# andrewendlinger/xmris

Hardware: AMD Instinct MI355X
Metric: spectra/sec (zero_fill->apodize->FFT->autophase), n_time=4096; HBM-roofline % (higher is better)
Workload: dtype f32

## Files before the change

xmris_amd/csrc/xm_coarse.h:

```cpp
#pragma once
#include "xm_kernels.h"

typedef _Float16 xm_h8 __attribute__((ext_vector_type(8)));
typedef _Float16 xm_h2 __attribute__((ext_vector_type(2)));
typedef float xm_f16v __attribute__((ext_vector_type(16)));

struct CoarseArgs {
  const void* in;
  const float* window;
  const Cx<float>* w1024;
  float* est;
  unsigned long long* gkey;
  long long in_stride;
  long long n_batch;
  float scale2;
};

constexpr int kCoarseWaves = 4;

XM_DEV Cx<float> coarse_w1024(const Cx<float>* __restrict__ t, unsigned k) {
  k &= 1023u;
  const Cx<float> w = t[k & 511u];
  return (k & 512u) ? mk<float>(-w.re, -w.im) : w;
}

XM_DEV xm_h8 coarse_pack(const float* v) {
  union {
    xm_h8 v8;
    xm_h2 v2[4];
  } u;
#pragma unroll
  for (int j = 0; j < 4; ++j) {
    const xm_f2 p = {v[2 * j], v[2 * j + 1]};
    u.v2[j] = __builtin_convertvector(p, xm_h2);
  }
  return u.v8;
}

template <bool IN64>
__global__ __launch_bounds__(64 * kCoarseWaves, 2) void k_coarse_mfma(CoarseArgs A) {
  const unsigned lane = threadIdx.x & 63u, r = lane & 31u, h = lane >> 5;
  const long long wave = (long long)blockIdx.x * kCoarseWaves + (threadIdx.x >> 6);
  const long long n_waves = (long long)gridDim.x * kCoarseWaves;

  xm_h8 b1r, b1i, b1n, a2r[2], a2i[2], a2n[2];
  {
    float cr[8], ci[8], cn[8];
#pragma unroll
    for (int j = 0; j < 8; ++j) {
      const Cx<float> w = coarse_w1024(A.w1024, 32u * ((8u * h + (unsigned)j) * r));
      cr[j] = w.re;
      ci[j] = w.im;
      cn[j] = -w.im;
    }
    b1r = coarse_pack(cr);
    b1i = coarse_pack(ci);
    b1n = coarse_pack(cn);
#pragma unroll
    for (int s = 0; s < 2; ++s) {
#pragma unroll
      for (int j = 0; j < 8; ++j) {
        const unsigned n2 = 16u * s + 8u * ((unsigned)j >> 2) + 4u * h + ((unsigned)j & 3u);
        const Cx<float> w = coarse_w1024(A.w1024, 32u * (n2 * r));
        cr[j] = w.re;
        ci[j] = w.im;
        cn[j] = -w.im;
      }
      a2r[s] = coarse_pack(cr);
      a2i[s] = coarse_pack(ci);
      a2n[s] = coarse_pack(cn);
    }
  }
  float twr[16], twi[16];
#pragma unroll
  for (int q = 0; q < 16; ++q) {
    const unsigned n2 = ((unsigned)q & 3u) + 8u * ((unsigned)q >> 2) + 4u * h;
    const Cx<float> w = coarse_w1024(A.w1024, n2 * r);
    twr[q] = w.re;
    twi[q] = w.im;
  }
  float wnd[8];
#pragma unroll
  for (int j = 0; j < 8; ++j) wnd[j] = A.window[32u * (8u * h + (unsigned)j) + r];

  auto fetch = [&](long long s, Cx<float>* x) {
    if constexpr (IN64) {
      const xm_d2* __restrict__ row = reinterpret_cast<const xm_d2*>(A.in) + s * A.in_stride;
#pragma unroll
      for (int j = 0; j < 8; ++j) {
        const xm_d2 v = __builtin_nontemporal_load(row + 32u * (8u * h + (unsigned)j) + r);
        x[j] = mk<float>((float)v.x, (float)v.y);
      }
      return;
    }
    const xm_f2* __restrict__ row = reinterpret_cast<const xm_f2*>(A.in) + s * A.in_stride;
#pragma unroll
    for (int j = 0; j < 8; ++j) {
      const xm_f2 v = __builtin_nontemporal_load(row + 32u * (8u * h + (unsigned)j) + r);
      x[j] = mk<float>(v.x, v.y);
    }
  };

  unsigned best_key = 0u, best_row = 0u;
  bool have = false;
  constexpr int DEPTH = 1;
  Cx<float> nx[DEPTH][8];
  long long s = wave;
#pragma unroll
  for (int d = 0; d < DEPTH; ++d)
    if (s + d * n_waves < A.n_batch) fetch(s + d * n_waves, nx[d]);
  auto one_row = [&](Cx<float>* cur, long long s) {
    float re[8], im[8];
    float m = 0.f;
#pragma unroll
    for (int j = 0; j < 8; ++j) {
      re[j] = cur[j].re * wnd[j];
      im[j] = cur[j].im * wnd[j];
      m = fmaxf(m, fmaxf(fabsf(re[j]), fabsf(im[j])));
    }
    if (s + DEPTH * n_waves < A.n_batch) fetch(s + DEPTH * n_waves, cur);
    unsigned e = (wave_reduce_u32<true>(__float_as_uint(m)) >> 23) & 0xffu;
    e = e > 253u ? 253u : (e < 1u ? 1u : e);
    const float up = __uint_as_float((254u - e) << 23);
    const float down = __uint_as_float(e << 23);
#pragma unroll
    for (int j = 0; j < 8; ++j) {
      re[j] *= up;
      im[j] *= up;
    }
    const xm_h8 ar = coarse_pack(re), ai = coarse_pack(im);
    xm_f16v d1r = {0.f}, d1i = {0.f};
    d1r = __builtin_amdgcn_mfma_f32_32x32x16_f16(ar, b1r, d1r, 0, 0, 0);
    d1r = __builtin_amdgcn_mfma_f32_32x32x16_f16(ai, b1n, d1r, 0, 0, 0);
    d1i = __builtin_amdgcn_mfma_f32_32x32x16_f16(ar, b1i, d1i, 0, 0, 0);
    d1i = __builtin_amdgcn_mfma_f32_32x32x16_f16(ai, b1r, d1i, 0, 0, 0);
    float zr[16], zi[16];
#pragma unroll
    for (int q = 0; q < 16; ++q) {
      zr[q] = d1r[q] * twr[q] - d1i[q] * twi[q];
      zi[q] = d1r[q] * twi[q] + d1i[q] * twr[q];
    }
    xm_f16v d2r = {0.f}, d2i = {0.f};
#pragma unroll
    for (int k = 0; k < 2; ++k) {
      const xm_h8 br = coarse_pack(zr + 8 * k), bi = coarse_pack(zi + 8 * k);
      d2r = __builtin_amdgcn_mfma_f32_32x32x16_f16(a2r[k], br, d2r, 0, 0, 0);
      d2r = __builtin_amdgcn_mfma_f32_32x32x16_f16(a2n[k], bi, d2r, 0, 0, 0);
      d2i = __builtin_amdgcn_mfma_f32_32x32x16_f16(a2r[k], bi, d2i, 0, 0, 0);
      d2i = __builtin_amdgcn_mfma_f32_32x32x16_f16(a2i[k], br, d2i, 0, 0, 0);
    }
    float bv = -1.f;
#pragma unroll
    for (int q = 0; q < 16; ++q) bv = fmaxf(bv, d2r[q] * d2r[q] + d2i[q] * d2i[q]);
    bv = amax_nan_if_unset(bv);
    bv = bv * (down * down) * A.scale2;
    const unsigned key = wave_reduce_u32<true>(bv != bv ? 0x7fc00000u : __float_as_uint(bv));
    const unsigned row = (unsigned)s;
    const bool take = !have || key > best_key;
    best_key = take ? key : best_key;
    best_row = take ? row : best_row;
    have = true;
    if (lane == 0u) A.est[s] = __uint_as_float(key);
  };
  for (; s < A.n_batch; s += DEPTH * n_waves) {
#pragma unroll
    for (int d = 0; d < DEPTH; ++d)
      if (s + d * n_waves < A.n_batch) one_row(nx[d], s + d * n_waves);
  }
  if (A.gkey && have && lane == 0u)
    atomicMax(A.gkey + (blockIdx.x % XM_KEY_SLOTS) * XM_KEY_STRIDE,
              ((unsigned long long)best_key << 32) | (unsigned long long)(0xffffffffu - best_row));
}
```

xmris_amd/csrc/xm_zf2p.h:

```cpp
#pragma once
#include "xm_kernels.h"

enum { ZF2P_LOAD16 = 1, ZF2P_NT = 2, ZF2P_QUEUE = 8, ZF2P_EST = 16, ZF2P_CAND = 32, ZF2P_IN64 = 64 };
constexpr int ZF2P_CAND_CAP = 16;
constexpr int ZF2P_CAND_KMAX = 16384;
constexpr int ZF2P_CAND_ROWS = 1, ZF2P_CAND_EST = 1 + ZF2P_CAND_CAP, ZF2P_CAND_COUNT = 1 + 2 * ZF2P_CAND_CAP,
              ZF2P_CAND_TOP = ZF2P_CAND_COUNT + 1, ZF2P_CAND_BITMAP = ZF2P_CAND_TOP + 1;
constexpr size_t zf2p_cand_lds_bytes() { return (ZF2P_CAND_BITMAP + ZF2P_CAND_KMAX / 32) * sizeof(unsigned); }

constexpr int xm_ilog2(int v) {
  int s = 0;
  while ((1 << s) < v) ++s;
  return s;
}

template <class PL, bool L16>
constexpr int zf2p_pad_shift() {
  if (!L16) return -1;
  return PL::radix(0) == 8 ? 4 : xm_ilog2(2 * PL::radix(0));
}

template <class PL, int MODE, int OPT>
__global__ __launch_bounds__(PL::NT, (zf2_waves<float, PL>())) void k_zf2p(PipeArgs<float> A) {
  using T = float;
  using V = xm_f2;
  constexpr unsigned N = 2 * PL::N, NT = PL::NT;
  constexpr int P = PL::P;
  constexpr bool WRITE = (MODE & ZF2_WRITE) != 0, PHASE = (MODE & ZF2_PHASE) != 0, AMAX = (MODE & ZF2_AMAX) != 0;
  constexpr bool RAMP = (MODE & ZF2_RAMP) != 0;
  constexpr bool L16 = (OPT & ZF2P_LOAD16) != 0;
  constexpr int AUX = (OPT & ZF2P_NT) ? 2 : 0;
  constexpr bool EST = (OPT & ZF2P_EST) != 0, CAND = (OPT & ZF2P_CAND) != 0, IN64 = (OPT & ZF2P_IN64) != 0;
  static_assert(!EST || (NT == XM_WAVE && AMAX && !WRITE), "the per-row estimate is stored by the row's one wave");
  static_assert(!CAND || (AMAX && !WRITE && (OPT & ZF2P_QUEUE) == 0), "candidates: maxima only, static order");
  static_assert(!(IN64 && L16), "pair loads are complex64 loads");
  static_assert(!(PHASE && RAMP), "phase table and ramp are exclusive");
  static_assert(!RAMP || WRITE, "a ramp needs an output");
  static_assert(P % 2 == 0 && NT >= XM_WAVE, "pair loads need an even number of points per thread, whole waves");
  using FFT = BlockFFT<V, PL, zf2p_pad_shift<PL, L16>()>;
  using HT = HotTw<T, PL, RAMP>;
  extern __shared__ __attribute__((aligned(16))) char xm_smem[];
  Cx<V>* lds = reinterpret_cast<Cx<V>*>(xm_smem);
  Cx<T>* mid = reinterpret_cast<Cx<T>*>(lds + FFT::lds_elems());
  T* red_v = reinterpret_cast<T*>(mid + HT::mid_lds_size());
  int* red_i = reinterpret_cast<int*>(red_v + NT / XM_WAVE + 1);
  unsigned* lds_next = reinterpret_cast<unsigned*>(red_i + NT / XM_WAVE + 1);
  constexpr bool QUEUE = (OPT & ZF2P_QUEUE) != 0;
  const unsigned t = threadIdx.x;
  const unsigned lane = t & (XM_WAVE - 1), half = lane >> 5;
  const unsigned col = L16 ? (t & ~(XM_WAVE - 1u)) + 2u * (lane & 31u) + half : t;

  long long n_rows = A.n_batch;
  unsigned* cand = lds_next + ZF2P_CAND_ROWS;
  const unsigned n_in = (unsigned)A.n_in;
  if constexpr (CAND) {
    float* cand_e = reinterpret_cast<float*>(lds_next + ZF2P_CAND_EST);
    unsigned* cand_n = lds_next + ZF2P_CAND_COUNT;
    unsigned* top_bits = lds_next + ZF2P_CAND_TOP;
    unsigned* bitmap = lds_next + ZF2P_CAND_BITMAP;
    const unsigned G = gridDim.x, b = blockIdx.x;
    const unsigned kmax = (unsigned)((A.n_batch + G - 1) / G);
    for (unsigned i = t; i < (kmax + 31u) / 32u; i += NT) bitmap[i] = 0u;
    if (t < XM_WAVE) {
      const unsigned long long k = __hip_atomic_load(A.gkey_in + t * XM_KEY_STRIDE, __ATOMIC_RELAXED, __HIP_MEMORY_SCOPE_AGENT);
      const unsigned hi = wave_reduce_u32<true>((unsigned)(k >> 32));
      if (t == 0) *top_bits = hi;
    }
    __syncthreads();
    const float thr = A.band2 * __uint_as_float(*top_bits);
    for (unsigned k = t; k < kmax; k += NT) {
      const long long r = (long long)k * G + (b + 37u * k) % G;
      if (r < A.n_batch) {
        const float e = A.est[r];
        if (e >= thr || e != e) atomicOr(&bitmap[k >> 5], 1u << (k & 31u));
      }
    }
    __syncthreads();
    if (t == 0) {
      unsigned n = 0;
      for (unsigned w = 0; w < (kmax + 31u) / 32u; ++w) {
        unsigned bits = bitmap[w];
        while (bits) {
          const unsigned k = w * 32u + (unsigned)__builtin_ctz(bits);
          bits &= bits - 1u;
          const unsigned r = (unsigned)((long long)k * G + (b + 37u * k) % G);
          float e = A.est[r];
          e = e != e ? __builtin_inff() : e;
// ... 8 lines not shown
          cand[pos] = r;
          cand_e[pos] = e;
          n = n < (unsigned)ZF2P_CAND_CAP ? n + 1u : n;
        }
      }
      *cand_n = n;
    }
    __syncthreads();
    n_rows = (long long)(unsigned)__builtin_amdgcn_readfirstlane((int)*cand_n);
  }
  const bool live = !CAND || n_rows > 0;

  HT tw;
  tw.mid = HT::mid_in_lds() ? mid : A.tw;
  if (live) {
    tw.load(A.tw, (int)t);
    for (unsigned i = t; i < (unsigned)HT::mid_lds_size(); i += NT) mid[i] = A.tw[i];
  }
  if constexpr (RAMP) {
    double sn, cs;
    sincos(A.ramp_db * (double)(2u * t), &sn, &cs);
    tw.fold(mk<T>((T)cs, (T)sn));
  }
  Cx<T> rot = live ? A.aux[col] : mk<T>(T(0), T(0));
  if constexpr (RAMP) rot = rot * mk<T>(A.ramp_e[0], A.ramp_e[1]);
  const unsigned coff = col - (unsigned)A.pad_left;
  T w[P];
#pragma unroll
  for (int q = 0; q < P; ++q) {
    const bool ok = live && (coff + NT * q) < n_in;
    w[q] = ok ? (A.window ? A.window[col + NT * q] * A.scale : A.scale) : T(0);
  }
  __syncthreads();

  constexpr int NRAW = L16 ? P / 2 : P;
  typedef unsigned raw_t __attribute__((ext_vector_type((L16 || IN64) ? 4 : 2)));
  raw_t raw[NRAW];
  const unsigned e0 = (t & ~(XM_WAVE - 1u)) + 2u * (lane & 31u) + NT * half - (unsigned)A.pad_left;
  auto fetch = [&](long long s2, unsigned ee0, unsigned cc, unsigned nin) {
    constexpr size_t EB = IN64 ? 16u : 8u;
    const char* __restrict__ row = reinterpret_cast<const char*>(A.in) + (size_t)(s2 * A.in_stride) * EB;
    if constexpr (L16) {
#pragma unroll
      for (int j = 0; j < P / 2; ++j) {
        const unsigned e = min(ee0 + 2u * NT * j, nin - 2u);
        raw[j] = __builtin_nontemporal_load(reinterpret_cast<const raw_t*>(row + (size_t)e * 8u));
      }
    } else {
#pragma unroll
      for (int q = 0; q < P; ++q) {
        const unsigned e = min(cc + NT * q, nin - 1u);
        raw[q] = *reinterpret_cast<const raw_t*>(row + (size_t)e * EB);
      }
    }
  };
  unsigned best_key = 0, best_row = 0;
  bool have = false;
  auto rowid = [&](long long v) -> long long {
    if constexpr (CAND) return (long long)(unsigned)__builtin_amdgcn_readfirstlane((int)cand[v]);
    else return v;
  };
  unsigned gb_seen = 0;
  auto next_live = [&](long long v) -> long long {
    if constexpr (CAND) {
      const float* cand_e = reinterpret_cast<const float*>(lds_next + ZF2P_CAND_EST);
      const unsigned gb = wave_reduce_u32<true>(__hip_atomic_load(A.gbest + lane * (2u * XM_KEY_STRIDE), __ATOMIC_RELAXED,
                                                                  __HIP_MEMORY_SCOPE_AGENT));
      gb_seen = gb;
      const float lim = A.band2 * __uint_as_float(gb);
      while (v < n_rows && __uint_as_float((unsigned)__builtin_amdgcn_readfirstlane((int)__float_as_uint(cand_e[v]))) < lim) ++v;
    }
    return v;
  };
  const long long ch = (!CAND && A.queue_chunk > 0) ? A.queue_chunk : 1;
  const long long c_first = CAND ? 0 : blockIdx.x, c_step = CAND ? 1 : gridDim.x;
  long long c_cur = c_first, c_nxt = c_cur + c_step, c_nn = c_nxt + c_step;
  long long s = c_cur * ch;
  unsigned off = 0;
  if constexpr (CAND) {
    if (n_rows > 0) {
      const float* cand_e = reinterpret_cast<const float*>(lds_next + ZF2P_CAND_EST);
      const float top = __uint_as_float((unsigned)__builtin_amdgcn_readfirstlane((int)__float_as_uint(cand_e[0])));
      const float emax2 = __uint_as_float((unsigned)__builtin_amdgcn_readfirstlane((int)lds_next[ZF2P_CAND_TOP]));
      if (top < 0.81f * emax2) {
#pragma unroll 1
        for (int i = 0; i < 3; ++i) __builtin_amdgcn_s_sleep(127);
        if (t < XM_WAVE) {
          const long long nx = next_live(0);
          if (t == 0u) *lds_next = (unsigned)nx;
        }
        __syncthreads();
        s = (long long)(unsigned)__builtin_amdgcn_readfirstlane((int)*lds_next);
        __syncthreads();
      }
    }
  }
  if (s < n_rows) fetch(rowid(s), e0, coff, n_in);
  if constexpr (QUEUE) {
    if (t == 0) *lds_next = atomicAdd(A.queue, 1u) + gridDim.x;
    __syncthreads();
    c_nxt = (long long)(unsigned)__builtin_amdgcn_readfirstlane((int)*lds_next);
    __syncthreads();
  }

  while (s < n_rows) {
    const bool chunk_end = (off + 1 == (unsigned)ch) || (s + 1 >= n_rows);
    long long s_nxt = chunk_end ? c_nxt * ch : s + 1;
    unsigned tt = t, cc = col, sh = (unsigned)A.out_shift, nin = n_in, pl = (unsigned)A.pad_left, ee0 = e0;
    asm volatile("" : "+v"(tt));
    asm volatile("" : "+v"(cc));
    asm volatile("" : "+v"(ee0));
    asm volatile("" : "+s"(sh));
    asm volatile("" : "+s"(nin));
    asm volatile("" : "+s"(pl));

    Cx<T> xr[P];
    if constexpr (L16) {
#pragma unroll
      for (int j = 0; j < P / 2; ++j) {
        const auto re = __builtin_amdgcn_permlane32_swap(raw[j].x, raw[j].z, false, false);
        const auto im = __builtin_amdgcn_permlane32_swap(raw[j].y, raw[j].w, false, false);
        xr[2 * j] = mk<T>(__uint_as_float(re[0]), __uint_as_float(im[0]));
        xr[2 * j + 1] = mk<T>(__uint_as_float(re[1]), __uint_as_float(im[1]));
      }
    } else if constexpr (IN64) {
#pragma unroll
      for (int q = 0; q < P; ++q) {
        Cx<double> d;
        __builtin_memcpy(&d, &raw[q], 16);
        xr[q] = mk<T>((T)d.re, (T)d.im);
      }
    } else {
#pragma unroll
      for (int q = 0; q < P; ++q) xr[q] = mk<T>(__uint_as_float(raw[q].x), __uint_as_float(raw[q].y));
    }
    Cx<V> v[P];
    static_for<0, P>([&](auto qc) {
      constexpr int q = decltype(qc)::value;
      const Cx<T> e = xr[q] * w[q];
      const Cx<T> o = mul_w<q, 2 * P, T>(e * rot);
      v[q].re = V{e.re, o.re};
      v[q].im = V{e.im, o.im};
    });
    if constexpr (!CAND) {
      if (s_nxt < n_rows) fetch(rowid(s_nxt), ee0, cc - pl, nin);
    }
    if constexpr (CAND) {
      FFT::run_cols(v, lds, tw, (int)tt, (int)cc, [&]() {
        if (tt < XM_WAVE) {
          const long long nx = next_live(s + 1);
          if (tt == 0u) *lds_next = (unsigned)nx;
        }
      });
      s_nxt = (long long)(unsigned)__builtin_amdgcn_readfirstlane((int)*lds_next);
      if (s_nxt < n_rows) fetch(rowid(s_nxt), ee0, cc - pl, nin);
    } else if constexpr (QUEUE) {
      const bool claim = off == 0u;
      unsigned ticket = 0;
      if (claim && tt == 0u) ticket = atomicAdd(A.queue, 1u) + gridDim.x;
      FFT::run_cols(v, lds, tw, (int)tt, (int)cc, [&]() {
        if (claim && tt == 0u) *lds_next = ticket;
      });
      if (claim) c_nn = (long long)(unsigned)__builtin_amdgcn_readfirstlane((int)*lds_next);
    } else {
      FFT::run_cols(v, lds, tw, (int)tt, (int)cc);
    }

    const unsigned t2 = 2u * tt;
    if constexpr (AMAX) {
// ... 153 lines not shown
```

xmris_amd/csrc/xm_launch_zf2p.hip:

```cpp
#include "xm_host.h"
#include "xm_plans.h"
#include "xm_tables.h"
#include "xm_zf2p.h"
#include "xm_coarse.h"

#include <cmath>
#include <cstdlib>
#include <cstring>
#include <mutex>

namespace {

using T = float;

template <class PL, int MODE, int OPT>
int launch_mode(PipeArgs<T> A, hipStream_t st) {
  const void* tw = nullptr;
  int rc = xm_table_get(TK_TWIDDLE, PL::N, PL::signature(), XM_C64, xm_gen_twiddles<PL>, nullptr, &tw);
  if (rc) return rc;
  A.tw = (const Cx<T>*)tw;
  if (A.n_batch <= 0) return XM_OK;
  constexpr bool L16 = (OPT & ZF2P_LOAD16) != 0;
  using FFT = BlockFFT<xm_f2, PL, zf2p_pad_shift<PL, L16>()>;
  constexpr bool CAND = (OPT & ZF2P_CAND) != 0;
// ... 42 lines not shown
  return xm_with_mode<W | R | AM, W | R, W | P | AM, W | P, W | AM, W, AM>(mode, [&](auto m) {
    constexpr int MODE = decltype(m)::value;
    return launch_mode<PL, MODE, (MODE & W) ? kOptWrite : kOptAmax>(A, st);
  });
}

}

namespace {

constexpr int kGuessHalf = 512;

template <class PL, bool IN64>
int launch_refine(const PipeArgs<T>& A, hipStream_t st) {
  return launch_mode<PL, ZF2_AMAX, ZF2P_CAND | (IN64 ? ZF2P_IN64 : ZF2P_LOAD16)>(A, st);
}

template <bool IN64>
int refine_plan(int h, const PipeArgs<T>& A, hipStream_t st) {
  switch (h) {
    case 512: return launch_refine<typename Zf2PlanOf<512>::type, IN64>(A, st);
    case 1024: return launch_refine<typename Zf2PlanOf<1024>::type, IN64>(A, st);
    case 2048: return launch_refine<typename Zf2PlanOf<2048>::type, IN64>(A, st);
    case 4096: return launch_refine<typename PlanOf<4096>::type, IN64>(A, st);
    case 8192: return launch_refine<typename Zf2PlanOf<8192>::type, IN64>(A, st);
    default: break;
  }
  return xm_fail(XM_ERR_UNSUPPORTED_N, "no half-length plan for " + std::to_string(h));
}

int half_table(int n, const Cx<T>** out) {
  const void* half = nullptr;
  const int rc = xm_table_get(TK_HALF, n, 0, XM_C64, xm_gen_half, nullptr, &half);
  *out = (const Cx<T>*)half;
  return rc;
}

}

int xm_zf2p_guess_supported(const void* in, int64_t in_stride, int n_in, int n_out, int pad_left, unsigned flags, int dtype) {
  const int h = n_out / 2;
  if (n_out % 2 || pad_left != 0 || n_in > h || n_in < 2) return 0;
  if (h != 512 && h != 1024 && h != 2048 && h != 4096 && h != 8192) return 0;
  if (flags & (XM_FFT_SHIFT_IN | XM_FFT_INVERSE)) return 0;
  if (dtype == XM_C128) return (reinterpret_cast<size_t>(in) & 15u) == 0;
  const int ng = n_in < kGuessHalf ? n_in : kGuessHalf;
  return xm_pair_loads_ok(in, in_stride, n_in, 0) && ng % 2 == 0;
}

int xm_zf2p_guess_rows(const void* in, int64_t in_stride, const float* window, int64_t n_batch, int n_in, int n_out,
                       int n_guess, float scale, float* est, unsigned long long* key, int dtype, hipStream_t st) {
  PipeArgs<T> A;
  std::memset(&A, 0, sizeof(A));
  A.in = (const Cx<T>*)in;
  A.window = window;
  A.in_stride = in_stride;
  A.n_batch = n_batch;
  A.n = 2 * kGuessHalf;
  int ng = n_guess > 0 && n_guess < kGuessHalf ? n_guess : kGuessHalf;
  if (ng > n_in) ng = n_in;
  if (dtype == XM_C64) ng &= ~1;
  A.n_in = ng;
  A.amax_value_only = 1;
  A.scale = scale;
  A.gkey = key;
  A.est = est;
  A.absmax2 = est;
  (void)n_out;
  int rc = half_table(A.n, &A.aux);
  if (rc) return rc;
  if (ng == kGuessHalf && window) {
    if (n_batch <= 0) return XM_OK;
    CoarseArgs C;
    C.in = in;
    C.window = window;
    C.w1024 = A.aux;
    C.est = est;
    C.gkey = key;
    C.in_stride = in_stride;
    C.n_batch = n_batch;
    C.scale2 = scale * scale;
    static XmResidency res32, res64;
    int resident = 0;
    rc = dtype == XM_C64 ? xm_resident_blocks(res32, k_coarse_mfma<false>, 64 * kCoarseWaves, 0, &resident, st)
                         : xm_resident_blocks(res64, k_coarse_mfma<true>, 64 * kCoarseWaves, 0, &resident, st);
    if (rc) return rc;
    const long long want = (n_batch + kCoarseWaves - 1) / kCoarseWaves;
    const long long blocks = want < resident ? want : resident;
    xm_note_kernel("k_coarse_mfma", nullptr, dtype == XM_C64 ? "float" : "double", kGuessHalf, -1);
    if (dtype == XM_C64)
      hipLaunchKernelGGL(k_coarse_mfma<false>, dim3((unsigned)blocks), dim3(64 * kCoarseWaves), 0, st, C);
    else
      hipLaunchKernelGGL(k_coarse_mfma<true>, dim3((unsigned)blocks), dim3(64 * kCoarseWaves), 0, st, C);
    HIP_TRY(hipGetLastError());
    return XM_OK;
  }
  using PL = typename Zf2PlanOf<kGuessHalf>::type;
  return dtype == XM_C64 ? launch_mode<PL, ZF2_AMAX, ZF2P_EST | ZF2P_LOAD16>(A, st)
                         : launch_mode<PL, ZF2_AMAX, ZF2P_EST | ZF2P_IN64>(A, st);
}

int xm_zf2p_guess_refine(const void* in, int64_t in_stride, const float* window, int64_t n_batch, int n_in, int n_out,
                         unsigned flags, float scale, const float* est, unsigned long long* guess_key, float band,
                         unsigned long long* work_key, float* out_max2, long long* out_flat, void* out_row, int dtype,
                         hipStream_t st) {
  PipeArgs<T> A;
  std::memset(&A, 0, sizeof(A));
  A.in = (const Cx<T>*)in;
  A.window = window;
  A.in_stride = in_stride;
  A.n_batch = n_batch;
  A.n = n_out;
  A.n_in = n_in;
  A.out_shift = (flags & XM_FFT_SHIFT_OUT) ? n_out / 2 : 0;
  A.amax_value_only = 1;
  A.scale = scale;
  A.gkey = work_key;
  A.gbest = reinterpret_cast<unsigned*>(work_key) + XM_KEY_GBEST_WORD;
  A.gkey_in = guess_key;
  A.est = const_cast<float*>(est);
  A.absmax2 = const_cast<float*>(est);
  A.band2 = band * band;
  A.take_max2 = out_max2;
  A.take_flat = out_flat;
  A.take_row = (Cx<double>*)out_row;
  int rc = half_table(n_out, &A.aux);
  if (rc) return rc;
  return dtype == XM_C64 ? refine_plan<false>(n_out / 2, A, st) : refine_plan<true>(n_out / 2, A, st);
}

int xm_zf2p_launch(int h, int mode, const PipeArgs<float>& A, const double* ramp, hipStream_t st) {
  switch (h) {
    case 512: return launch_plan<typename Zf2PlanOf<512>::type>(A, mode, ramp, st);
    case 1024: return launch_plan<typename Zf2PlanOf<1024>::type>(A, mode, ramp, st);
    case 2048: return launch_plan<typename Zf2PlanOf<2048>::type>(A, mode, ramp, st);
    case 4096: return launch_plan<typename PlanOf<4096>::type>(A, mode, ramp, st);
    case 8192: return launch_plan<typename Zf2PlanOf<8192>::type>(A, mode, ramp, st);
    default: break;
  }
  return xm_fail(XM_ERR_UNSUPPORTED_N, "no half-length plan for " + std::to_string(h));
}
```

Baseline: 57.17 million.

## Vectorize coarse-estimate loads, deepen prefetch, and batch estimate stores

The coarse MFMA estimator now loads f32 input rows as 16-byte vectors and uses permlane16_swap plus a permuted index mapping (sigma/n1) to redistribute elements into the layout the MFMA stages expect. Prefetch depth rises from one to two rows, with clamped fetches and a validity flag in place of per-row branches. Per-row estimate stores from lane 0 are collected in lanes and written as one block. The intent is fewer, wider memory transactions, more loads in flight, and fewer scattered stores, at the cost of more registers and extra permutation logic in the index mapping.

```diff
diff --git a/xmris_amd/csrc/xm_coarse.h b/xmris_amd/csrc/xm_coarse.h
--- a/xmris_amd/csrc/xm_coarse.h
+++ b/xmris_amd/csrc/xm_coarse.h
@@ -17,6 +17,11 @@
 };
 
 constexpr int kCoarseWaves = 4;
+constexpr int kCoarseDepth = 2;
+constexpr bool kCoarseNT = true;
+
+XM_DEV constexpr unsigned coarse_sigma(unsigned i) { return 2u * (i & 15u) + (i >> 4); }
+XM_DEV constexpr unsigned coarse_n1(unsigned h, unsigned u) { return 4u * (u >> 1) + 2u * h + (u & 1u); }
 
 XM_DEV Cx<float> coarse_w1024(const Cx<float>* __restrict__ t, unsigned k) {
   k &= 1023u;
@@ -38,9 +43,22 @@
 }
 
 template <bool IN64>
+struct CoarseRaw {
+  typedef xm_u4 type;
+  static constexpr int n = 4;
+};
+template <>
+struct CoarseRaw<true> {
+  typedef xm_d2 type;
+  static constexpr int n = 8;
+};
+
+template <bool IN64>
 __global__ __launch_bounds__(64 * kCoarseWaves, 2) void k_coarse_mfma(CoarseArgs A) {
+  using raw_t = typename CoarseRaw<IN64>::type;
+  constexpr int NRAW = CoarseRaw<IN64>::n;
   const unsigned lane = threadIdx.x & 63u, r = lane & 31u, h = lane >> 5;
-  const long long wave = (long long)blockIdx.x * kCoarseWaves + (threadIdx.x >> 6);
+  const long long wave = (long long)blockIdx.x * kCoarseWaves + __builtin_amdgcn_readfirstlane((int)(threadIdx.x >> 6));
   const long long n_waves = (long long)gridDim.x * kCoarseWaves;
 
   xm_h8 b1r, b1i, b1n, a2r[2], a2i[2], a2n[2];
@@ -48,7 +66,7 @@
     float cr[8], ci[8], cn[8];
 #pragma unroll
     for (int j = 0; j < 8; ++j) {
-      const Cx<float> w = coarse_w1024(A.w1024, 32u * ((8u * h + (unsigned)j) * r));
+      const Cx<float> w = coarse_w1024(A.w1024, 32u * (coarse_n1(h, (unsigned)j) * r));
       cr[j] = w.re;
       ci[j] = w.im;
       cn[j] = -w.im;
@@ -60,7 +78,7 @@
     for (int s = 0; s < 2; ++s) {
 #pragma unroll
       for (int j = 0; j < 8; ++j) {
-        const unsigned n2 = 16u * s + 8u * ((unsigned)j >> 2) + 4u * h + ((unsigned)j & 3u);
+        const unsigned n2 = coarse_sigma(16u * s + 8u * ((unsigned)j >> 2) + 4u * h + ((unsigned)j & 3u));
         const Cx<float> w = coarse_w1024(A.w1024, 32u * (n2 * r));
         cr[j] = w.re;
         ci[j] = w.im;
@@ -74,51 +92,67 @@
   float twr[16], twi[16];
 #pragma unroll
   for (int q = 0; q < 16; ++q) {
-    const unsigned n2 = ((unsigned)q & 3u) + 8u * ((unsigned)q >> 2) + 4u * h;
+    const unsigned n2 = coarse_sigma(((unsigned)q & 3u) + 8u * ((unsigned)q >> 2) + 4u * h);
     const Cx<float> w = coarse_w1024(A.w1024, n2 * r);
     twr[q] = w.re;
     twi[q] = w.im;
   }
+  const unsigned n2own = coarse_sigma(r);
   float wnd[8];
 #pragma unroll
-  for (int j = 0; j < 8; ++j) wnd[j] = A.window[32u * (8u * h + (unsigned)j) + r];
-
-  auto fetch = [&](long long s, Cx<float>* x) {
+  for (int u = 0; u < 8; ++u) wnd[u] = A.window[32u * coarse_n1(h, (unsigned)u) + n2own];
+
+  auto ld = [](const raw_t* p) -> raw_t {
+    if constexpr (kCoarseNT) return __builtin_nontemporal_load(p);
+    else return *p;
+  };
+  auto fetch = [&](long long s, raw_t* x) {
+    s = s < A.n_batch ? s : A.n_batch - 1;
     if constexpr (IN64) {
-      const xm_d2* __restrict__ row = reinterpret_cast<const xm_d2*>(A.in) + s * A.in_stride;
-#pragma unroll
-      for (int j = 0; j < 8; ++j) {
-        const xm_d2 v = __builtin_nontemporal_load(row + 32u * (8u * h + (unsigned)j) + r);
-        x[j] = mk<float>((float)v.x, (float)v.y);
-      }
-      return;
-    }
-    const xm_f2* __restrict__ row = reinterpret_cast<const xm_f2*>(A.in) + s * A.in_stride;
-#pragma unroll
-    for (int j = 0; j < 8; ++j) {
-      const xm_f2 v = __builtin_nontemporal_load(row + 32u * (8u * h + (unsigned)j) + r);
-      x[j] = mk<float>(v.x, v.y);
+      const xm_d2* __restrict__ row = reinterpret_cast<const xm_d2*>(A.in) + s * A.in_stride + n2own;
+#pragma unroll
+      for (int u = 0; u < 8; ++u) x[u] = ld(row + 32u * coarse_n1(h, (unsigned)u));
+    } else {
+      const xm_u4* __restrict__ row =
+          reinterpret_cast<const xm_u4*>(reinterpret_cast<const xm_f2*>(A.in) + s * A.in_stride) + lane;
+#pragma unroll
+      for (int j = 0; j < 4; ++j) x[j] = ld(row + 64u * j);
     }
   };
 
   unsigned best_key = 0u, best_row = 0u;
   bool have = false;
-  constexpr int DEPTH = 1;
-  Cx<float> nx[DEPTH][8];
-  long long s = wave;
-#pragma unroll
-  for (int d = 0; d < DEPTH; ++d)
-    if (s + d * n_waves < A.n_batch) fetch(s + d * n_waves, nx[d]);
-  auto one_row = [&](Cx<float>* cur, long long s) {
+  constexpr int DEPTH = kCoarseDepth;
+  constexpr unsigned BLK = (64 / DEPTH) * DEPTH;
+  const long long n_mine = wave < A.n_batch ? (A.n_batch - wave + n_waves - 1) / n_waves : 0;
+  unsigned keep = 0u, slot = 0u;
+  raw_t nx[DEPTH][NRAW];
+#pragma unroll
+  for (int d = 0; d < DEPTH; ++d) fetch(wave + d * n_waves, nx[d]);
+  auto one_row = [&](raw_t* cur, long long s, bool valid) {
     float re[8], im[8];
+    if constexpr (IN64) {
+#pragma unroll
+      for (int u = 0; u < 8; ++u) {
+        re[u] = (float)cur[u].x * wnd[u];
+        im[u] = (float)cur[u].y * wnd[u];
+      }
+    } else {
+#pragma unroll
+      for (int j = 0; j < 4; ++j) {
+        const auto vr = __builtin_amdgcn_permlane16_swap(cur[j].x, cur[j].z, false, false);
+        const auto vi = __builtin_amdgcn_permlane16_swap(cur[j].y, cur[j].w, false, false);
+        re[2 * j] = __uint_as_float(vr[0]) * wnd[2 * j];
+        re[2 * j + 1] = __uint_as_float(vr[1]) * wnd[2 * j + 1];
+        im[2 * j] = __uint_as_float(vi[0]) * wnd[2 * j];
+        im[2 * j + 1] = __uint_as_float(vi[1]) * wnd[2 * j + 1];
+      }
+    }
+    fetch(s + DEPTH * n_waves, cur);
+    __builtin_amdgcn_sched_barrier(0);
     float m = 0.f;
 #pragma unroll
-    for (int j = 0; j < 8; ++j) {
-      re[j] = cur[j].re * wnd[j];
-      im[j] = cur[j].im * wnd[j];
-      m = fmaxf(m, fmaxf(fabsf(re[j]), fabsf(im[j])));
-    }
-    if (s + DEPTH * n_waves < A.n_batch) fetch(s + DEPTH * n_waves, cur);
+    for (int j = 0; j < 8; ++j) m = fmaxf(m, fmaxf(fabsf(re[j]), fabsf(im[j])));
     unsigned e = (wave_reduce_u32<true>(__float_as_uint(m)) >> 23) & 0xffu;
     e = e > 253u ? 253u : (e < 1u ? 1u : e);
     const float up = __uint_as_float((254u - e) << 23);
@@ -156,17 +190,28 @@
     bv = bv * (down * down) * A.scale2;
     const unsigned key = wave_reduce_u32<true>(bv != bv ? 0x7fc00000u : __float_as_uint(bv));
     const unsigned row = (unsigned)s;
-    const bool take = !have || key > best_key;
+    const bool take = valid && (!have || key > best_key);
     best_key = take ? key : best_key;
     best_row = take ? row : best_row;
-    have = true;
-    if (lane == 0u) A.est[s] = __uint_as_float(key);
-  };
-  for (; s < A.n_batch; s += DEPTH * n_waves) {
-#pragma unroll
-    for (int d = 0; d < DEPTH; ++d)
-      if (s + d * n_waves < A.n_batch) one_row(nx[d], s + d * n_waves);
-  }
+    have = have || valid;
+    keep = lane == slot ? key : keep;
+    ++slot;
+  };
+  auto store_block = [&](long long first) {
+    const long long left = n_mine - first;
+    if ((long long)lane < left && lane < slot) A.est[wave + (first + lane) * n_waves] = __uint_as_float(keep);
+    slot = 0u;
+  };
+  long long it = 0, first = 0;
+  for (; it < n_mine; it += DEPTH) {
+#pragma unroll
+    for (int d = 0; d < DEPTH; ++d) one_row(nx[d], wave + (it + d) * n_waves, it + d < n_mine);
+    if (slot == BLK) {
+      store_block(first);
+      first = it + DEPTH;
+    }
+  }
+  if (slot != 0u) store_block(first);
   if (A.gkey && have && lane == 0u)
     atomicMax(A.gkey + (blockIdx.x % XM_KEY_SLOTS) * XM_KEY_STRIDE,
               ((unsigned long long)best_key << 32) | (unsigned long long)(0xffffffffu - best_row));
diff --git a/xmris_amd/csrc/xm_zf2p.h b/xmris_amd/csrc/xm_zf2p.h
--- a/xmris_amd/csrc/xm_zf2p.h
+++ b/xmris_amd/csrc/xm_zf2p.h
@@ -3,6 +3,7 @@
 
 enum { ZF2P_LOAD16 = 1, ZF2P_NT = 2, ZF2P_QUEUE = 8, ZF2P_EST = 16, ZF2P_CAND = 32, ZF2P_IN64 = 64 };
 constexpr int ZF2P_CAND_CAP = 16;
+constexpr int ZF2P_CAND_NAP = 3;
 constexpr int ZF2P_CAND_KMAX = 16384;
 constexpr int ZF2P_CAND_ROWS = 1, ZF2P_CAND_EST = 1 + ZF2P_CAND_CAP, ZF2P_CAND_COUNT = 1 + 2 * ZF2P_CAND_CAP,
               ZF2P_CAND_TOP = ZF2P_CAND_COUNT + 1, ZF2P_CAND_BITMAP = ZF2P_CAND_TOP + 1;
@@ -177,9 +178,9 @@
       const float* cand_e = reinterpret_cast<const float*>(lds_next + ZF2P_CAND_EST);
       const float top = __uint_as_float((unsigned)__builtin_amdgcn_readfirstlane((int)__float_as_uint(cand_e[0])));
       const float emax2 = __uint_as_float((unsigned)__builtin_amdgcn_readfirstlane((int)lds_next[ZF2P_CAND_TOP]));
-      if (top < 0.81f * emax2) {
+      if (ZF2P_CAND_NAP > 0 && top < 0.81f * emax2) {
 #pragma unroll 1
-        for (int i = 0; i < 3; ++i) __builtin_amdgcn_s_sleep(127);
+        for (int i = 0; i < ZF2P_CAND_NAP; ++i) __builtin_amdgcn_s_sleep(127);
         if (t < XM_WAVE) {
           const long long nx = next_live(0);
           if (t == 0u) *lds_next = (unsigned)nx;
```

After: 58.01 million (median of 4 runs). 1.5% higher.

## Move coarse-FFT DFT operands and twiddles to LDS and raise occupancy

Applied to the files above, without the earlier changes.

Per-lane DFT matrix operands, twiddles and window values were held in registers. They are now built once per block, split across the four waves, into shared memory, and reloaded from LDS inside each row. Launch bounds go from 2 to 4 blocks per CU, so more waves can be resident to hide the latency of the streaming loads. The twiddle multiply and magnitude reduction are also reshaped into paired products with asm barriers so that rounding matches a reference. This costs extra LDS reads on every row and adds a __syncthreads at kernel start.

```diff
diff --git a/xmris_amd/csrc/xm_coarse.h b/xmris_amd/csrc/xm_coarse.h
--- a/xmris_amd/csrc/xm_coarse.h
+++ b/xmris_amd/csrc/xm_coarse.h
@@ -4,6 +4,7 @@
 typedef _Float16 xm_h8 __attribute__((ext_vector_type(8)));
 typedef _Float16 xm_h2 __attribute__((ext_vector_type(2)));
 typedef float xm_f16v __attribute__((ext_vector_type(16)));
+typedef float xm_f4 __attribute__((ext_vector_type(4)));
 
 struct CoarseArgs {
   const void* in;
@@ -18,6 +19,16 @@
 
 constexpr int kCoarseWaves = 4;
 
+enum {
+  kCoarseB1 = 0,
+  kCoarseA2 = 3,
+  kCoarseHalfSlots = 9,
+  kCoarseTwr = 0,
+  kCoarseTwi = 4,
+  kCoarseWnd = 8,
+  kCoarseFloatSlots = 10,
+};
+
 XM_DEV Cx<float> coarse_w1024(const Cx<float>* __restrict__ t, unsigned k) {
   k &= 1023u;
   const Cx<float> w = t[k & 511u];
@@ -37,51 +48,63 @@
   return u.v8;
 }
 
+XM_DEV xm_f2 coarse_rounded(xm_f2 p) {
+  asm("" : "+v"(p));
+  return p;
+}
+
+template <class F>
+XM_DEV void coarse_w32_operands(const Cx<float>* __restrict__ w1024, unsigned r, F n_of, xm_h8* dst) {
+  float cr[8], ci[8], cn[8];
+#pragma unroll
+  for (int j = 0; j < 8; ++j) {
+    const Cx<float> w = coarse_w1024(w1024, 32u * (n_of((unsigned)j) * r));
+    cr[j] = w.re;
+    ci[j] = w.im;
+    cn[j] = -w.im;
+  }
+  dst[0 * XM_WAVE] = coarse_pack(cr);
+  dst[1 * XM_WAVE] = coarse_pack(ci);
+  dst[2 * XM_WAVE] = coarse_pack(cn);
+}
+
 template <bool IN64>
-__global__ __launch_bounds__(64 * kCoarseWaves, 2) void k_coarse_mfma(CoarseArgs A) {
+__global__ __launch_bounds__(64 * kCoarseWaves, 4) void k_coarse_mfma(CoarseArgs A) {
   const unsigned lane = threadIdx.x & 63u, r = lane & 31u, h = lane >> 5;
-  const long long wave = (long long)blockIdx.x * kCoarseWaves + (threadIdx.x >> 6);
+  const unsigned wv = threadIdx.x >> 6;
+  const long long wave = (long long)blockIdx.x * kCoarseWaves + wv;
   const long long n_waves = (long long)gridDim.x * kCoarseWaves;
-
-  xm_h8 b1r, b1i, b1n, a2r[2], a2i[2], a2n[2];
-  {
-    float cr[8], ci[8], cn[8];
-#pragma unroll
-    for (int j = 0; j < 8; ++j) {
-      const Cx<float> w = coarse_w1024(A.w1024, 32u * ((8u * h + (unsigned)j) * r));
-      cr[j] = w.re;
-      ci[j] = w.im;
-      cn[j] = -w.im;
-    }
-    b1r = coarse_pack(cr);
-    b1i = coarse_pack(ci);
-    b1n = coarse_pack(cn);
-#pragma unroll
-    for (int s = 0; s < 2; ++s) {
-#pragma unroll
-      for (int j = 0; j < 8; ++j) {
-        const unsigned n2 = 16u * s + 8u * ((unsigned)j >> 2) + 4u * h + ((unsigned)j & 3u);
-        const Cx<float> w = coarse_w1024(A.w1024, 32u * (n2 * r));
-        cr[j] = w.re;
-        ci[j] = w.im;
-        cn[j] = -w.im;
-      }
-      a2r[s] = coarse_pack(cr);
-      a2i[s] = coarse_pack(ci);
-      a2n[s] = coarse_pack(cn);
+  __shared__ xm_h8 c_half[kCoarseHalfSlots][XM_WAVE];
+  __shared__ xm_f4 c_float[kCoarseFloatSlots][XM_WAVE];
+
+  if (wv == 0u) {
+    coarse_w32_operands(A.w1024, r, [&](unsigned j) { return 8u * h + j; }, &c_half[kCoarseB1][lane]);
+#pragma unroll
+    for (int g = 0; g < 2; ++g) {
+      xm_f4 w;
+#pragma unroll
+      for (int j = 0; j < 4; ++j) w[j] = A.window[32u * (8u * h + 4u * g + (unsigned)j) + r];
+      c_float[kCoarseWnd + g][lane] = w;
+    }
+  } else if (wv < 3u) {
+    const unsigned s = wv - 1u;
+    coarse_w32_operands(A.w1024, r, [&](unsigned j) { return 16u * s + 8u * (j >> 2) + 4u * h + (j & 3u); },
+                        &c_half[kCoarseA2 + 3 * s][lane]);
+  } else {
+#pragma unroll
+    for (int g = 0; g < 4; ++g) {
+      xm_f4 wr, wi;
+#pragma unroll
+      for (int j = 0; j < 4; ++j) {
+        const Cx<float> w = coarse_w1024(A.w1024, ((unsigned)j + 8u * g + 4u * h) * r);
+        wr[j] = w.re;
+        wi[j] = w.im;
+      }
+      c_float[kCoarseTwr + g][lane] = wr;
+      c_float[kCoarseTwi + g][lane] = wi;
     }
   }
-  float twr[16], twi[16];
-#pragma unroll
-  for (int q = 0; q < 16; ++q) {
-    const unsigned n2 = ((unsigned)q & 3u) + 8u * ((unsigned)q >> 2) + 4u * h;
-    const Cx<float> w = coarse_w1024(A.w1024, n2 * r);
-    twr[q] = w.re;
-    twi[q] = w.im;
-  }
-  float wnd[8];
-#pragma unroll
-  for (int j = 0; j < 8; ++j) wnd[j] = A.window[32u * (8u * h + (unsigned)j) + r];
+  __syncthreads();
 
   auto fetch = [&](long long s, Cx<float>* x) {
     if constexpr (IN64) {
@@ -103,22 +126,26 @@
 
   unsigned best_key = 0u, best_row = 0u;
   bool have = false;
-  constexpr int DEPTH = 1;
-  Cx<float> nx[DEPTH][8];
+  Cx<float> nx[8];
   long long s = wave;
-#pragma unroll
-  for (int d = 0; d < DEPTH; ++d)
-    if (s + d * n_waves < A.n_batch) fetch(s + d * n_waves, nx[d]);
+  if (s < A.n_batch) fetch(s, nx);
   auto one_row = [&](Cx<float>* cur, long long s) {
+    unsigned ll = lane;
+    asm volatile("" : "+v"(ll));
     float re[8], im[8];
     float m = 0.f;
 #pragma unroll
-    for (int j = 0; j < 8; ++j) {
-      re[j] = cur[j].re * wnd[j];
-      im[j] = cur[j].im * wnd[j];
-      m = fmaxf(m, fmaxf(fabsf(re[j]), fabsf(im[j])));
-    }
-    if (s + DEPTH * n_waves < A.n_batch) fetch(s + DEPTH * n_waves, cur);
+    for (int g = 0; g < 2; ++g) {
+      const xm_f4 wnd = c_float[kCoarseWnd + g][ll];
+#pragma unroll
+      for (int i = 0; i < 4; ++i) {
+        const int j = 4 * g + i;
+        re[j] = cur[j].re * wnd[i];
+        im[j] = cur[j].im * wnd[i];
+        m = fmaxf(m, fmaxf(fabsf(re[j]), fabsf(im[j])));
+      }
+    }
+    if (s + n_waves < A.n_batch) fetch(s + n_waves, cur);
     unsigned e = (wave_reduce_u32<true>(__float_as_uint(m)) >> 23) & 0xffu;
     e = e > 253u ? 253u : (e < 1u ? 1u : e);
     const float up = __uint_as_float((254u - e) << 23);
@@ -130,28 +157,47 @@
     }
     const xm_h8 ar = coarse_pack(re), ai = coarse_pack(im);
     xm_f16v d1r = {0.f}, d1i = {0.f};
-    d1r = __builtin_amdgcn_mfma_f32_32x32x16_f16(ar, b1r, d1r, 0, 0, 0);
-    d1r = __builtin_amdgcn_mfma_f32_32x32x16_f16(ai, b1n, d1r, 0, 0, 0);
-    d1i = __builtin_amdgcn_mfma_f32_32x32x16_f16(ar, b1i, d1i, 0, 0, 0);
-    d1i = __builtin_amdgcn_mfma_f32_32x32x16_f16(ai, b1r, d1i, 0, 0, 0);
+    {
+      const xm_h8 b1r = c_half[kCoarseB1][ll], b1i = c_half[kCoarseB1 + 1][ll], b1n = c_half[kCoarseB1 + 2][ll];
+      d1r = __builtin_amdgcn_mfma_f32_32x32x16_f16(ar, b1r, d1r, 0, 0, 0);
+      d1r = __builtin_amdgcn_mfma_f32_32x32x16_f16(ai, b1n, d1r, 0, 0, 0);
+      d1i = __builtin_amdgcn_mfma_f32_32x32x16_f16(ar, b1i, d1i, 0, 0, 0);
+      d1i = __builtin_amdgcn_mfma_f32_32x32x16_f16(ai, b1r, d1i, 0, 0, 0);
+    }
     float zr[16], zi[16];
 #pragma unroll
-    for (int q = 0; q < 16; ++q) {
-      zr[q] = d1r[q] * twr[q] - d1i[q] * twi[q];
-      zi[q] = d1r[q] * twi[q] + d1i[q] * twr[q];
+    for (int g = 0; g < 4; ++g) {
+      const xm_f4 twr = c_float[kCoarseTwr + g][ll], twi = c_float[kCoarseTwi + g][ll];
+#pragma unroll
+      for (int i = 0; i < 4; i += 2) {
+        const int q = 4 * g + i;
+        const xm_f2 ii = coarse_rounded(xm_f2{d1i[q] * twi[i], d1i[q + 1] * twi[i + 1]});
+        const xm_f2 ri = coarse_rounded(xm_f2{d1r[q] * twi[i], d1r[q + 1] * twi[i + 1]});
+        zr[q] = __builtin_fmaf(d1r[q], twr[i], -ii.x);
+        zr[q + 1] = __builtin_fmaf(d1r[q + 1], twr[i + 1], -ii.y);
+        zi[q] = __builtin_fmaf(d1i[q], twr[i], ri.x);
+        zi[q + 1] = __builtin_fmaf(d1i[q + 1], twr[i + 1], ri.y);
+      }
     }
     xm_f16v d2r = {0.f}, d2i = {0.f};
 #pragma unroll
     for (int k = 0; k < 2; ++k) {
       const xm_h8 br = coarse_pack(zr + 8 * k), bi = coarse_pack(zi + 8 * k);
-      d2r = __builtin_amdgcn_mfma_f32_32x32x16_f16(a2r[k], br, d2r, 0, 0, 0);
-      d2r = __builtin_amdgcn_mfma_f32_32x32x16_f16(a2n[k], bi, d2r, 0, 0, 0);
-      d2i = __builtin_amdgcn_mfma_f32_32x32x16_f16(a2r[k], bi, d2i, 0, 0, 0);
-      d2i = __builtin_amdgcn_mfma_f32_32x32x16_f16(a2i[k], br, d2i, 0, 0, 0);
+      const xm_h8 a2r = c_half[kCoarseA2 + 3 * k][ll], a2i = c_half[kCoarseA2 + 3 * k + 1][ll],
+                  a2n = c_half[kCoarseA2 + 3 * k + 2][ll];
+      d2r = __builtin_amdgcn_mfma_f32_32x32x16_f16(a2r, br, d2r, 0, 0, 0);
+      d2r = __builtin_amdgcn_mfma_f32_32x32x16_f16(a2n, bi, d2r, 0, 0, 0);
+      d2i = __builtin_amdgcn_mfma_f32_32x32x16_f16(a2r, bi, d2i, 0, 0, 0);
+      d2i = __builtin_amdgcn_mfma_f32_32x32x16_f16(a2i, br, d2i, 0, 0, 0);
     }
     float bv = -1.f;
 #pragma unroll
-    for (int q = 0; q < 16; ++q) bv = fmaxf(bv, d2r[q] * d2r[q] + d2i[q] * d2i[q]);
+    for (int q = 0; q < 16; q += 2) {
+      const xm_f2 ii = coarse_rounded(xm_f2{d2i[q] * d2i[q], d2i[q + 1] * d2i[q + 1]});
+      const xm_f2 rr = coarse_rounded(xm_f2{d2r[q] * d2r[q], d2r[q + 1] * d2r[q + 1]});
+      bv = fmaxf(bv, q < 5 ? __builtin_fmaf(d2r[q], d2r[q], ii.x) : rr.x + ii.x);
+      bv = fmaxf(bv, q + 1 < 5 ? __builtin_fmaf(d2r[q + 1], d2r[q + 1], ii.y) : rr.y + ii.y);
+    }
     bv = amax_nan_if_unset(bv);
     bv = bv * (down * down) * A.scale2;
     const unsigned key = wave_reduce_u32<true>(bv != bv ? 0x7fc00000u : __float_as_uint(bv));
@@ -162,11 +208,7 @@
     have = true;
     if (lane == 0u) A.est[s] = __uint_as_float(key);
   };
-  for (; s < A.n_batch; s += DEPTH * n_waves) {
-#pragma unroll
-    for (int d = 0; d < DEPTH; ++d)
-      if (s + d * n_waves < A.n_batch) one_row(nx[d], s + d * n_waves);
-  }
+  for (; s < A.n_batch; s += n_waves) one_row(nx, s);
   if (A.gkey && have && lane == 0u)
     atomicMax(A.gkey + (blockIdx.x % XM_KEY_SLOTS) * XM_KEY_STRIDE,
               ((unsigned long long)best_key << 32) | (unsigned long long)(0xffffffffu - best_row));
```

Measured after the change: 58.56 million before, 58.83 million after (median of 6 runs). No clear change (+0.5%).

## Stream coarse-guess rows through an LDS ring with direct global-to-LDS loads

Applied to the files above, without the earlier changes.

For complex64 input, the coarse MFMA guess kernel no longer does a register prefetch of depth one. Each wave now issues global_load_lds_dwordx4 loads into a per-wave LDS ring of several rows and waits on vmcnt, so multiple rows stay in flight while earlier ones are transformed. Per-row estimate stores are gathered across lanes and flushed as one coalesced 64-wide write instead of one scalar store per row. This adds 64 KiB of dynamic LDS per block, which can cut occupancy, and it relies on inline assembly that manipulates m0 and the waitcnt counters.

```diff
diff --git a/xmris_amd/csrc/xm_coarse.h b/xmris_amd/csrc/xm_coarse.h
--- a/xmris_amd/csrc/xm_coarse.h
+++ b/xmris_amd/csrc/xm_coarse.h
@@ -17,6 +17,27 @@
 };
 
 constexpr int kCoarseWaves = 4;
+constexpr int kCoarseRow = 512;
+
+#ifndef XM_COARSE_RING
+#define XM_COARSE_RING 4
+#endif
+#ifndef XM_COARSE_POLICY
+#define XM_COARSE_POLICY " nt"
+#endif
+constexpr int kCoarseRowBytes = kCoarseRow * 8;
+constexpr size_t kCoarseLdsBytes = (size_t)kCoarseWaves * XM_COARSE_RING * kCoarseRowBytes;
+static_assert(XM_COARSE_RING >= 2 && kCoarseLdsBytes <= 65536, "ring of the coarse spectra: 2 rows ... 64 KiB");
+
+typedef __attribute__((address_space(3))) char xm_lds_byte;
+
+template <int G, int MAXR>
+XM_DEV void coarse_wait_rows(long long rows) {
+  if (rows >= MAXR)
+    asm volatile("s_waitcnt vmcnt(%0)" ::"n"(G * MAXR) : "memory");
+  else if constexpr (MAXR > 0)
+    coarse_wait_rows<G, MAXR - 1>(rows);
+}
 
 XM_DEV Cx<float> coarse_w1024(const Cx<float>* __restrict__ t, unsigned k) {
   k &= 1023u;
@@ -40,7 +61,8 @@
 template <bool IN64>
 __global__ __launch_bounds__(64 * kCoarseWaves, 2) void k_coarse_mfma(CoarseArgs A) {
   const unsigned lane = threadIdx.x & 63u, r = lane & 31u, h = lane >> 5;
-  const long long wave = (long long)blockIdx.x * kCoarseWaves + (threadIdx.x >> 6);
+  const unsigned wid = __builtin_amdgcn_readfirstlane(threadIdx.x >> 6);
+  const long long wave = (long long)blockIdx.x * kCoarseWaves + wid;
   const long long n_waves = (long long)gridDim.x * kCoarseWaves;
 
   xm_h8 b1r, b1i, b1n, a2r[2], a2i[2], a2n[2];
@@ -83,33 +105,47 @@
 #pragma unroll
   for (int j = 0; j < 8; ++j) wnd[j] = A.window[32u * (8u * h + (unsigned)j) + r];
 
-  auto fetch = [&](long long s, Cx<float>* x) {
-    if constexpr (IN64) {
-      const xm_d2* __restrict__ row = reinterpret_cast<const xm_d2*>(A.in) + s * A.in_stride;
-#pragma unroll
-      for (int j = 0; j < 8; ++j) {
-        const xm_d2 v = __builtin_nontemporal_load(row + 32u * (8u * h + (unsigned)j) + r);
-        x[j] = mk<float>((float)v.x, (float)v.y);
-      }
-      return;
-    }
-    const xm_f2* __restrict__ row = reinterpret_cast<const xm_f2*>(A.in) + s * A.in_stride;
-#pragma unroll
-    for (int j = 0; j < 8; ++j) {
-      const xm_f2 v = __builtin_nontemporal_load(row + 32u * (8u * h + (unsigned)j) + r);
+  constexpr int RING = XM_COARSE_RING;
+  extern __shared__ __attribute__((aligned(16))) char xm_smem[];
+  const unsigned ring0 = (unsigned)(unsigned long)(xm_lds_byte*)xm_smem + wid * (unsigned)(RING * kCoarseRowBytes);
+  auto issue = [&](long long s, unsigned slot) {
+    const unsigned char* src = reinterpret_cast<const unsigned char*>(A.in) + s * A.in_stride * 8 + 16u * lane;
+    const unsigned dst = __builtin_amdgcn_readfirstlane(ring0 + slot * (unsigned)kCoarseRowBytes);
+    unsigned keep;
+    asm volatile(
+        "s_waitcnt lgkmcnt(0)\n\t"
+        "s_mov_b32 %0, m0\n\t"
+        "s_mov_b32 m0, %2\n\t"
+        "s_nop 0\n\t"
+        "global_load_lds_dwordx4 %1, off" XM_COARSE_POLICY "\n\t"
+        "global_load_lds_dwordx4 %1, off offset:1024" XM_COARSE_POLICY "\n\t"
+        "global_load_lds_dwordx4 %1, off offset:2048" XM_COARSE_POLICY "\n\t"
+        "global_load_lds_dwordx4 %1, off offset:3072" XM_COARSE_POLICY "\n\t"
+        "s_mov_b32 m0, %0"
+        : "=&s"(keep)
+        : "v"(src), "s"(dst)
+        : "memory");
+  };
+  auto take = [&](unsigned slot, Cx<float>* x) {
+    const xm_f2* row = reinterpret_cast<const xm_f2*>(xm_smem + (wid * (unsigned)RING + slot) * (unsigned)kCoarseRowBytes);
+#pragma unroll
+    for (int j = 0; j < 8; ++j) {
+      const xm_f2 v = row[32u * (8u * h + (unsigned)j) + r];
       x[j] = mk<float>(v.x, v.y);
+    }
+  };
+  auto fetch64 = [&](long long s, Cx<float>* x) {
+    const xm_d2* __restrict__ row = reinterpret_cast<const xm_d2*>(A.in) + s * A.in_stride;
+#pragma unroll
+    for (int j = 0; j < 8; ++j) {
+      const xm_d2 v = __builtin_nontemporal_load(row + 32u * (8u * h + (unsigned)j) + r);
+      x[j] = mk<float>((float)v.x, (float)v.y);
     }
   };
 
   unsigned best_key = 0u, best_row = 0u;
   bool have = false;
-  constexpr int DEPTH = 1;
-  Cx<float> nx[DEPTH][8];
-  long long s = wave;
-#pragma unroll
-  for (int d = 0; d < DEPTH; ++d)
-    if (s + d * n_waves < A.n_batch) fetch(s + d * n_waves, nx[d]);
-  auto one_row = [&](Cx<float>* cur, long long s) {
+  auto one_row = [&](const Cx<float>* cur, long long s, auto&& windowed) -> unsigned {
     float re[8], im[8];
     float m = 0.f;
 #pragma unroll
@@ -118,7 +154,7 @@
       im[j] = cur[j].im * wnd[j];
       m = fmaxf(m, fmaxf(fabsf(re[j]), fabsf(im[j])));
     }
-    if (s + DEPTH * n_waves < A.n_batch) fetch(s + DEPTH * n_waves, cur);
+    windowed();
     unsigned e = (wave_reduce_u32<true>(__float_as_uint(m)) >> 23) & 0xffu;
     e = e > 253u ? 253u : (e < 1u ? 1u : e);
     const float up = __uint_as_float((254u - e) << 23);
@@ -156,16 +192,44 @@
     bv = bv * (down * down) * A.scale2;
     const unsigned key = wave_reduce_u32<true>(bv != bv ? 0x7fc00000u : __float_as_uint(bv));
     const unsigned row = (unsigned)s;
-    const bool take = !have || key > best_key;
-    best_key = take ? key : best_key;
-    best_row = take ? row : best_row;
+    const bool better = !have || key > best_key;
+    best_key = better ? key : best_key;
+    best_row = better ? row : best_row;
     have = true;
-    if (lane == 0u) A.est[s] = __uint_as_float(key);
-  };
-  for (; s < A.n_batch; s += DEPTH * n_waves) {
-#pragma unroll
-    for (int d = 0; d < DEPTH; ++d)
-      if (s + d * n_waves < A.n_batch) one_row(nx[d], s + d * n_waves);
+    return key;
+  };
+
+  if constexpr (IN64) {
+    Cx<float> nx[8];
+    long long s = wave;
+    if (s < A.n_batch) fetch64(s, nx);
+    for (; s < A.n_batch; s += n_waves) {
+      const unsigned key = one_row(nx, s, [&] {
+        if (s + n_waves < A.n_batch) fetch64(s + n_waves, nx);
+      });
+      if (lane == 0u) A.est[s] = __uint_as_float(key);
+    }
+  } else {
+    const long long mine = wave < A.n_batch ? (A.n_batch - wave + n_waves - 1) / n_waves : 0;
+    auto flush = [&](long long k0, unsigned held) {
+      if (k0 + (long long)lane < mine) A.est[wave + (k0 + (long long)lane) * n_waves] = __uint_as_float(held);
+    };
+#pragma unroll
+    for (int d = 0; d < RING; ++d)
+      if (d < mine) issue(wave + d * n_waves, (unsigned)d);
+    unsigned slot = 0u, held = 0u;
+    for (long long k = 0; k < mine; ++k) {
+      const long long left = mine - 1 - k;
+      coarse_wait_rows<4, RING - 1>(left);
+      Cx<float> x[8];
+      take(slot, x);
+      if (k + RING < mine) issue(wave + (k + RING) * n_waves, slot);
+      const unsigned key = one_row(x, wave + k * n_waves, [] {});
+      held = ((unsigned)k & 63u) == lane ? key : held;
+      if (((unsigned)k & 63u) == 63u) flush(k - 63, held);
+      slot = slot + 1u == (unsigned)RING ? 0u : slot + 1u;
+    }
+    if (mine & 63) flush(mine & ~63ll, held);
   }
   if (A.gkey && have && lane == 0u)
     atomicMax(A.gkey + (blockIdx.x % XM_KEY_SLOTS) * XM_KEY_STRIDE,
diff --git a/xmris_amd/csrc/xm_launch_zf2p.hip b/xmris_amd/csrc/xm_launch_zf2p.hip
--- a/xmris_amd/csrc/xm_launch_zf2p.hip
+++ b/xmris_amd/csrc/xm_launch_zf2p.hip
@@ -148,14 +148,14 @@
     C.scale2 = scale * scale;
     static XmResidency res32, res64;
     int resident = 0;
-    rc = dtype == XM_C64 ? xm_resident_blocks(res32, k_coarse_mfma<false>, 64 * kCoarseWaves, 0, &resident, st)
+    rc = dtype == XM_C64 ? xm_resident_blocks(res32, k_coarse_mfma<false>, 64 * kCoarseWaves, kCoarseLdsBytes, &resident, st)
                          : xm_resident_blocks(res64, k_coarse_mfma<true>, 64 * kCoarseWaves, 0, &resident, st);
     if (rc) return rc;
     const long long want = (n_batch + kCoarseWaves - 1) / kCoarseWaves;
     const long long blocks = want < resident ? want : resident;
     xm_note_kernel("k_coarse_mfma", nullptr, dtype == XM_C64 ? "float" : "double", kGuessHalf, -1);
     if (dtype == XM_C64)
-      hipLaunchKernelGGL(k_coarse_mfma<false>, dim3((unsigned)blocks), dim3(64 * kCoarseWaves), 0, st, C);
+      hipLaunchKernelGGL(k_coarse_mfma<false>, dim3((unsigned)blocks), dim3(64 * kCoarseWaves), kCoarseLdsBytes, st, C);
     else
       hipLaunchKernelGGL(k_coarse_mfma<true>, dim3((unsigned)blocks), dim3(64 * kCoarseWaves), 0, st, C);
     HIP_TRY(hipGetLastError());
```

After: 58.09 million before, 58.44 million after (median of 3 runs). Within noise of the previous version (+0.6%).
